# Isomorpfishm/SINGA

Measured on AMD Instinct MI355X. Metric: protein-ligand graphs/sec GAN step (G+D fwd+bwd); scatter-TP kernel HBM GB/s, higher is better.
Workload: dtype f32

## Files before the change

### __graft_entry__.py

```python
import os
import subprocess
import sys

ROOT = os.path.dirname(os.path.abspath(__file__))
if ROOT not in sys.path:
    sys.path.insert(0, ROOT)

SRC = os.path.join(ROOT, "singa_amd", "csrc", "singa_hip.hip")
LIB = os.path.join(ROOT, "singa_amd", "lib", "libsinga_hip.so")


def build() -> None:
    os.makedirs(os.path.dirname(LIB), exist_ok=True)
    deps = [SRC, os.path.join(ROOT, "singa_amd", "csrc", "so3_index.h"), os.path.join(ROOT, "include", "singa_hip.h"),
            os.path.join(ROOT, "include", "singa_hip_lab.h"), os.path.join(ROOT, "include", "singa_hip_gen.h"),
            os.path.join(ROOT, "include", "singa_hip_force.h"), os.path.join(ROOT, "include", "singa_hip_swor.h"),
            os.path.join(ROOT, "include", "singa_hip_stream.h"), os.path.join(ROOT, "include", "singa_hip_valence.h"),
            os.path.join(ROOT, "include", "singa_hip_beam.h")]
    if not os.path.exists(LIB) or any(os.path.getmtime(d) > os.path.getmtime(LIB) for d in deps):
        hipcc = os.environ.get("HIPCC", "/opt/rocm/bin/hipcc")
        cmd = [hipcc, "--offload-arch=gfx950", "-O3", "-std=c++17", "-shared", "-fPIC", "-o", LIB, SRC]
        subprocess.check_call(cmd)
    import torch
    import singa_amd
    from singa_amd import _capi
    _capi.bind(LIB)


def smoke() -> None:
    import numpy as np
    import torch

    build()
    from oracle import singa_oracle as O
    from singa_amd import graph as G
    from singa_amd.config import load_config
    from singa_amd.model.GAN import SINGA
    from tests.helpers import golden, state_from_spec

    assert torch.cuda.is_available(), "smoke() needs a GPU"
    L = 2
    dev = "cuda:0"
    sd = state_from_spec(f"singa_L{L}")
    z = golden(f"singa_L{L}_B3.npz")
    names = ["3wi2_4tpp", "4agq_5a7b", "5cp5_4nue"]
    batch = G.collate([G.load_npz(os.path.join(ROOT, "tests", "golden", f"graph_{n}.npz"), with_lap=False) for n in names])
    batch.nodes[G.PA]["lap_pe"], batch.nodes[G.LA]["lap_pe"] = torch.tensor(z["lap_p"]), torch.tensor(z["lap_l"])
    batch.extras["edge_rot_mat"] = {k: torch.tensor(z[f"rot_{k}"]) for k in ("pp", "ll", "lp")}
    batch.extras["knn"] = {G.PA: torch.tensor(z["knn_p"]), G.LA: torch.tensor(z["knn_l"])}
    batch = batch.to(dev)
    model = SINGA(load_config(lmax=L), device=dev)
    model.load_state_dict(sd, strict=False)
    model.eval()
    logits = model(batch)
    loss = torch.nn.functional.cross_entropy(logits, batch["ligand_data"]["smiIndices_tgt"].reshape(-1))
    loss.backward()
    torch.cuda.synchronize()
    og = O.collate([O.load_graph_npz(os.path.join(ROOT, "tests", "golden", f"graph_{n}.npz")) for n in names])
    rots = {k: torch.as_tensor(z[f"rot_{k}"]) for k in ("pp", "ll", "lp")}
    with torch.no_grad():
        ref = O.singa_forward(sd, og, rots, L, torch.as_tensor(z["knn_p"]), torch.as_tensor(z["knn_l"]),
                              torch.as_tensor(z["lap_p"]), torch.as_tensor(z["lap_l"]))
    err = float((logits.detach().cpu().double() - ref.double()).norm() / ref.double().norm())
    gn = float(torch.sqrt(sum((p.grad.double() ** 2).sum() for p in model.parameters() if p.grad is not None)))
    print(f"smoke: loss {float(loss):.6f} (reference {float(z['loss']):.6f}), logits rel err vs oracle {err:.2e}, "
          f"grad norm {gn:.4f} (reference {float(z['grad_total']):.4f})")
    assert err < 1e-4, err
    assert abs(gn - float(z["grad_total"])) < 1e-4 * float(z["grad_total"])


if __name__ == "__main__":
# ... 4 lines not shown
```

### singa_amd/_capi.py

```python
import ctypes as C

P = C.c_void_p
I32 = C.c_int
I64 = C.c_int64
F32 = C.c_float


class Seg(C.Structure):
    _fields_ = [("ptr", P), ("ld", I64), ("rows", C.c_int32)]


SegArr = Seg * 3


class Gemm(C.Structure):
    _fields_ = [("a", P), ("b", P), ("c", P), ("bias", P), ("lda", I64), ("ldb", I64), ("ldc", I64), ("I", C.c_int32),
                ("J", C.c_int32), ("R", C.c_int32), ("a_group", C.c_int32), ("b_group", C.c_int32), ("c_group", C.c_int32),
                ("a_group_ld", I64), ("b_group_ld", I64), ("c_group_ld", I64), ("c_split_stride", I64), ("mask", P),
                ("addend", P), ("relu", C.c_int32), ("asum", P), ("asum_stride", I64)]


class CGemm(C.Structure):
    _fields_ = [("a", P), ("b", P), ("c", P), ("lda", I64), ("ldb", I64), ("ldc", I64), ("a_im", I64), ("b_im", I64),
                ("c_im", I64), ("c_split_stride", I64), ("I", C.c_int32), ("J", C.c_int32), ("R", C.c_int32),
# ... 94 lines not shown

EXPORTS = tuple(_SIGS)

_LAB_SIGS = {
    "singa_so3_skinny_variant": ([I32], I32),
    "singa_gemm_occupancy": ([I32, I32, I32], I32),
    "singa_gemm_force_cfg": ([I32], I32),
    "singa_lap_pe_fsi_min": ([I32], I32),
}
LAB_EXPORTS = tuple(_LAB_SIGS)

_GEN_SIGS = {
    "singa_sample_token_grammar": ([P, P, P, P, P, I32, I32, I32, I32, F32, I32, F32, I32, I32] + [P] * 10, I32),
    "singa_smiles_rule_host": ([P, P, P, I32, P, P], I32),
}
GEN_EXPORTS = tuple(_GEN_SIGS)

_FORCE_SIGS = {
    "singa_sample_token_forced": ([P, P, P, P, P, I32, I32, I32, I32, F32, I32, F32, I32, I32] + [P] * 12, I32),
}
FORCE_EXPORTS = tuple(_FORCE_SIGS)

U64 = C.c_uint64
_SWOR_SIGS = {
    "singa_swor_noise_host": ([U64, P, P, P, I32, P, P, P], I32),
    "singa_swor_work": ([I32, I32], C.c_longlong),
    "singa_swor_expand": ([P, P, P, P, I32, I32, I32, I32, I32, F32, U64, P, I32] + [P] * 8 + [P], I32),
    "singa_swor_select": ([P, P, P, P, P, I32, I32, I32, I32, I32, I32, I32] + [P] * 13 + [P], I32),
    "singa_swor_follow": ([P] * 8 + [I32] * 6 + [I64] * 4 + [P], I32),
}
SWOR_EXPORTS = tuple(_SWOR_SIGS)

_STREAM_SIGS = {
    "singa_dec_self_attn_rows": ([P] * 10 + [I32, I32, P, F32, P], I32),
    "singa_sample_token_stream": ([P] * 6 + [I32, I32, I32, I32, I32, F32, I32, F32, I32, I32] + [P] * 7 + [P], I32),
    "singa_stream_refill": ([I32] * 8 + [P] * 8 + [P], I32),
    "singa_stream_refill_host": ([I32] * 8 + [P] * 8, I32),
}
STREAM_EXPORTS = tuple(_STREAM_SIGS)

_VALENCE_SIGS = {
    "singa_sample_token_valence": ([P] * 7 + [I32, I32, I32, I32, I32, F32, I32, F32, I32, I32] + [P] * 12 + [P], I32),
    "singa_valence_rule_host": ([P] * 5 + [I32] + [P] * 3, I32),
}
VALENCE_EXPORTS = tuple(_VALENCE_SIGS)

_BEAM_SIGS = {
    "singa_beam_work": ([I32, I32], C.c_longlong),
    "singa_beam_expand": ([P] * 5 + [I32] * 5 + [P] * 5 + [P], I32),
    "singa_beam_select": ([P] * 4 + [I32] * 7 + [P] * 18 + [P], I32),
}
BEAM_EXPORTS = tuple(_BEAM_SIGS)


def bind(path):
    import torch
    lib = C.CDLL(path)
    for name, (args, res) in list(_SIGS.items()) + list(_LAB_SIGS.items()) + list(_GEN_SIGS.items()) + \
            list(_FORCE_SIGS.items()) + list(_SWOR_SIGS.items()) + list(_STREAM_SIGS.items()) + list(_VALENCE_SIGS.items()) + \
            list(_BEAM_SIGS.items()):
        fn = getattr(lib, name)
        fn.argtypes = args
        fn.restype = res
    return lib


def segs(items):
    arr = SegArr()
    for i, (p, ld, rows) in enumerate(items):
        arr[i].ptr, arr[i].ld, arr[i].rows = p, ld, rows
    return arr, len(items)


def check(lib, code, what):
    if code != 0:
        raise RuntimeError(f"{what} failed ({code}): {lib.singa_last_error_string().decode()}")
```

### singa_amd/csrc/singa_hip.hip

```cpp
#include <hip/hip_runtime.h>
#include <hip/hip_ext.h>

#include <math.h>
#include <stdint.h>
#include <stdio.h>
#include <string.h>
#include <type_traits>

#include "../../include/singa_hip.h"
#include "../../include/singa_hip_lab.h"
#include "../../include/singa_hip_gen.h"
#include "../../include/singa_hip_force.h"
#include "../../include/singa_hip_swor.h"
#include "../../include/singa_hip_stream.h"
#include "../../include/singa_hip_valence.h"
#include "../../include/singa_hip_beam.h"
#include "so3_index.h"

namespace {

thread_local char g_err[256] = "ok";

int fail(int code, const char* msg) {
    snprintf(g_err, sizeof(g_err), "%s", msg);
    return code;
}

int check_launch(const char* what) {
    hipError_t e = hipGetLastError();
    if (e != hipSuccess) {
        snprintf(g_err, sizeof(g_err), "%s: %s", what, hipGetErrorString(e));
        return (int)e;
    }
    return SINGA_OK;
}

struct ProfRec {
    hipEvent_t a, b;
    int E, N, tag;
};
constexpr int PROF_CAP = 8192;
ProfRec g_prof[PROF_CAP];
int g_prof_n = 0;
bool g_prof_on = false;
unsigned long long* g_stamp_buf = nullptr;
int g_stamp_cap = 0;
__global__ void stamp_kernel(unsigned long long* dst) { *dst = (unsigned long long)wall_clock64(); }
int g_prof_edges_hint = 0;

#ifndef SINGA_KEEP_VGPR
#define SINGA_KEEP_VGPR(x) __asm__ volatile("" : "+v"(x))
#endif

#define SINGA_LAUNCH(tag_, E_, N_, kern, grid, block, st, ...)                                                   \
    do {                                                                                                          \
        if (g_prof_on && g_prof_n < PROF_CAP) {                                                                   \
            ProfRec& r_ = g_prof[g_prof_n++];                                                                     \
            (void)hipEventCreate(&r_.a);                                                                          \
            (void)hipEventCreate(&r_.b);                                                                          \
            r_.E = (E_);                                                                                          \
            r_.N = (N_);                                                                                          \
            r_.tag = (tag_);                                                                                      \
            hipExtLaunchKernelGGL(kern, grid, block, 0, (st), r_.a, r_.b, 0, __VA_ARGS__);                        \
        } else if (g_stamp_buf && 2 * (g_prof_n + 2) <= g_stamp_cap && g_prof_n + 1 < PROF_CAP) {                 \
            if (g_prof_n == 0) {                                                                                  \
                g_prof[0].a = g_prof[0].b = nullptr;                                                              \
                g_prof[0].E = g_prof[0].N = g_prof[0].tag = 0;                                                    \
                hipLaunchKernelGGL(stamp_kernel, dim3(1), dim3(1), 0, (st), g_stamp_buf);                         \
                hipLaunchKernelGGL(stamp_kernel, dim3(1), dim3(1), 0, (st), g_stamp_buf + 1);                     \
// ... 5712 lines not shown
    return SINGA_OK;
}

template <int MAXC>
__global__ __launch_bounds__(256) void knn_graph_kernel(const float* __restrict__ pos, const int* __restrict__ batch,
                                                        const long long* __restrict__ ptr, int B, int N, int k,
                                                        long long* __restrict__ row, long long* __restrict__ col) {
    const int lane = threadIdx.x & 63;
    const int i = blockIdx.x * (blockDim.x >> 6) + (threadIdx.x >> 6);
    if (i >= N) return;
    const int g = batch[i];
    long long* ro = row + (long long)i * k;
    long long* co = col + (long long)i * k;
    if (g < 0 || g >= B) {
        for (int r = lane; r < k; r += 64) ro[r] = co[r] = -1;
        return;
    }
    const int lo = (int)ptr[g], hi = (int)ptr[g + 1];
    const float px = pos[3 * i], py = pos[3 * i + 1], pz = pos[3 * i + 2];
    const unsigned long long NONE = ~0ull;
    unsigned long long key[MAXC];
#pragma unroll
    for (int t = 0; t < MAXC; ++t) {
        const int c = lo + lane + 64 * t;
        key[t] = NONE;
        if (c < hi && c != i) {
            const float dx = __fsub_rn(px, pos[3 * c]), dy = __fsub_rn(py, pos[3 * c + 1]), dz = __fsub_rn(pz, pos[3 * c + 2]);
            const float d2 = __fadd_rn(__fadd_rn(__fmul_rn(dx, dx), __fmul_rn(dy, dy)), __fmul_rn(dz, dz));
            key[t] = ((unsigned long long)__float_as_uint(d2) << 32) | (unsigned)c;
        }
    }
    for (int r = 0; r < k; ++r) {
        unsigned long long best = key[0];
#pragma unroll
        for (int t = 1; t < MAXC; ++t) best = key[t] < best ? key[t] : best;
#pragma unroll
        for (int o = 32; o > 0; o >>= 1) {
            const unsigned blo = (unsigned)__shfl_xor((int)(unsigned)best, o, 64);
            const unsigned bhi = (unsigned)__shfl_xor((int)(unsigned)(best >> 32), o, 64);
            const unsigned long long other = ((unsigned long long)bhi << 32) | blo;
            best = other < best ? other : best;
        }
#pragma unroll
        for (int t = 0; t < MAXC; ++t)
            if (key[t] == best) key[t] = NONE;
        if (lane == 0) {
            const bool have = best != NONE;
            ro[r] = have ? (long long)i : -1;
            co[r] = have ? (long long)(unsigned)best : -1;
        }
    }
}

__global__ void calib_copy_kernel(const float* __restrict__ src, float* __restrict__ dst, long long n) {
    long long i = (long long)blockIdx.x * blockDim.x + threadIdx.x;
    long long stride = (long long)gridDim.x * blockDim.x;
    for (; i < n; i += stride) dst[i] = src[i];
}

template <int UNROLL>
__global__ void __launch_bounds__(256) calib_copy16_kernel(const float4* __restrict__ src, float4* __restrict__ dst, long long n4) {
    const long long chunk = 256LL * UNROLL;
    for (long long base = (long long)blockIdx.x * chunk; base < n4; base += (long long)gridDim.x * chunk) {
        float4 v[UNROLL];
#pragma unroll
        for (int u = 0; u < UNROLL; ++u) {
            const long long i = base + threadIdx.x + 256LL * u;
            if (i < n4) v[u] = src[i];
        }
#pragma unroll
        for (int u = 0; u < UNROLL; ++u) {
            const long long i = base + threadIdx.x + 256LL * u;
            if (i < n4) dst[i] = v[u];
        }
    }
}

}

extern "C" {

int singa_prof_enable(int on) {
    g_prof_on = on != 0;
    return SINGA_OK;
}

int singa_prof_stamps(unsigned long long* buf, int cap) {
    g_stamp_buf = buf;
    g_stamp_cap = buf ? cap : 0;
    if (buf) {
        g_prof_on = false;
        g_prof_n = 0;
    }
    return SINGA_OK;
}

int singa_prof_read_stamps(const unsigned long long* host_stamps, float* ms, int* tags, int* edges, int* nodes, int cap) {
    if (!host_stamps) return 0;
    int n = 0;
    double calib = (double)(host_stamps[1] - host_stamps[0]);
    for (int i = 1; i < g_prof_n && n < cap; ++i) {
        double ticks = (double)(host_stamps[2 * i + 1] - host_stamps[2 * i]) - calib;
        ms[n] = (float)(ticks * 1e-5);
        tags[n] = g_prof[i].tag;
        edges[n] = g_prof[i].E;
        nodes[n] = g_prof[i].N;
// ... 26 lines not shown
        (void)hipEventDestroy(g_prof[i].a);
        (void)hipEventDestroy(g_prof[i].b);
    }
    g_prof_n = 0;
    return n;
}

int singa_prof_collect_tagged(float* ms, int* tags, int* edges, int* nodes, int cap) {
    int n = 0;
    for (int i = 0; i < g_prof_n; ++i) {
        float t = 0.f;
        hipError_t e = hipEventElapsedTime(&t, g_prof[i].a, g_prof[i].b);
        if (e == hipSuccess && n < cap) {
            ms[n] = t;
            tags[n] = g_prof[i].tag;
            edges[n] = g_prof[i].E;
            nodes[n] = g_prof[i].N;
            ++n;
        }
        (void)hipEventDestroy(g_prof[i].a);
        (void)hipEventDestroy(g_prof[i].b);
    }
    g_prof_n = 0;
    return n;
}

int singa_calib_copy(const float* src, float* dst, long long n, void* stream) {
    if (!src || !dst) return fail(SINGA_E_NULL, "calib_copy: null pointer");
    hipLaunchKernelGGL(calib_copy_kernel, dim3(256 * 8), dim3(256), 0, (hipStream_t)stream, src, dst, n);
    return check_launch("calib_copy");
}

int singa_knn_graph(const float* pos, const int32_t* batch, const long long* ptr, int B, int N, int k, int max_nodes, long long* row,
                    long long* col, void* stream) {
    if (!pos || !batch || !ptr || !row || !col) return fail(SINGA_E_NULL, "knn_graph: null pointer");
    if (B < 0 || N < 0 || k <= 0 || max_nodes < 0 || max_nodes > 2048) return fail(SINGA_E_SHAPE, "knn_graph: k > 0 and at most 2048 atoms per molecule");
    if (N == 0) return SINGA_OK;
    const dim3 grid((unsigned)((N + 3) / 4)), block(256);
    hipStream_t st = (hipStream_t)stream;
    if (max_nodes <= 512) hipLaunchKernelGGL(knn_graph_kernel<8>, grid, block, 0, st, pos, batch, ptr, B, N, k, row, col);
    else if (max_nodes <= 1024) hipLaunchKernelGGL(knn_graph_kernel<16>, grid, block, 0, st, pos, batch, ptr, B, N, k, row, col);
    else hipLaunchKernelGGL(knn_graph_kernel<32>, grid, block, 0, st, pos, batch, ptr, B, N, k, row, col);
    return check_launch("knn_graph");
}

int singa_knn_edge_attr(const float* len, const int32_t* ptr, long long n_real, const float* offset, float coeff, float* out, int N,
                        int G, void* stream) {
    if (!ptr || !offset || !out || (!len && n_real > 0)) return fail(SINGA_E_NULL, "knn_edge_attr: null pointer");
    if (G != 64) return fail(SINGA_E_SHAPE, "knn_edge_attr: 64 Gaussians (the shipped edge_channels)");
    if (N < 0 || n_real < 0) return fail(SINGA_E_SHAPE, "knn_edge_attr: negative size");
    if (N == 0) return SINGA_OK;
    hipLaunchKernelGGL(knn_edge_attr_kernel, dim3(kn_grid(N)), dim3(64), 0, (hipStream_t)stream, len, ptr, n_real, offset, coeff, out, N);
    return check_launch("knn_edge_attr");
}

int singa_calib_copy16(const float* src, float* dst, long long n, int blocks, int unroll, void* stream) {
    if (!src || !dst) return fail(SINGA_E_NULL, "calib_copy16: null pointer");
    if (n % 4 || ((uintptr_t)src | (uintptr_t)dst) % 16) return fail(SINGA_E_SHAPE, "calib_copy16: n % 4 == 0 and 16-byte aligned pointers");
    if (blocks < 1 || blocks > (1 << 20) || (unroll != 1 && unroll != 2 && unroll != 4 && unroll != 8))
        return fail(SINGA_E_SHAPE, "calib_copy16: blocks >= 1, unroll in {1, 2, 4, 8}");
    const float4* s4 = (const float4*)src;
    float4* d4 = (float4*)dst;
    hipStream_t st = (hipStream_t)stream;
    if (unroll == 1) hipLaunchKernelGGL(calib_copy16_kernel<1>, dim3(blocks), dim3(256), 0, st, s4, d4, n / 4);
    else if (unroll == 2) hipLaunchKernelGGL(calib_copy16_kernel<2>, dim3(blocks), dim3(256), 0, st, s4, d4, n / 4);
    else if (unroll == 4) hipLaunchKernelGGL(calib_copy16_kernel<4>, dim3(blocks), dim3(256), 0, st, s4, d4, n / 4);
    else hipLaunchKernelGGL(calib_copy16_kernel<8>, dim3(blocks), dim3(256), 0, st, s4, d4, n / 4);
    return check_launch("calib_copy16");
}

int singa_version(void) { return 100; }

const char* singa_last_error_string(void) { return g_err; }

int singa_init(const double* jd_flat, int lmax_max) {
    if (!jd_flat) return fail(SINGA_E_NULL, "singa_init: jd_flat is null");
    if (lmax_max < 0 || lmax_max > 11) return fail(SINGA_E_LMAX, "singa_init: lmax_max must be in [0, 11]");
    static float host[MAX_J];
    int n = j_off(lmax_max + 1);
    for (int i = 0; i < n; ++i) host[i] = (float)jd_flat[i];
    hipError_t e = hipMemcpyToSymbol(HIP_SYMBOL(g_J), host, n * sizeof(float), 0, hipMemcpyHostToDevice);
    if (e != hipSuccess) {
        snprintf(g_err, sizeof(g_err), "singa_init: %s", hipGetErrorString(e));
        return (int)e;
    }
    g_lmax_init = lmax_max;
    return SINGA_OK;
}

int singa_dims(int lmax, int mmax, int* kr, int* wsz, int* rad_rows) {
    SINGA_DISPATCH_L(lmax, mmax, {
        using I = SO3Idx<L_, 2>;
        if (kr) *kr = I::KR;
        if (wsz) *wsz = I::WSZ;
        if (rad_rows) *rad_rows = I::RAD_ROWS;
    });
    return SINGA_OK;
}

int singa_edge_frames(const float* vec, const float* rnd, float* rot, float* stats, int E, void* stream) {
    if (!vec || !rnd || !rot || !stats) return fail(SINGA_E_NULL, "edge_frames: null pointer");
    if (E <= 0) return SINGA_OK;
    hipLaunchKernelGGL(edge_frames_kernel, dim3((E + 255) / 256), dim3(256), 0, (hipStream_t)stream, vec, rnd, rot,
                       (int*)stats, E);
    return check_launch("edge_frames");
}
// ... 1463 lines not shown
```

### singa_amd/model/CProMG.py

```python
import math
import os

import numpy as np
import torch
import torch.nn as nn
import torch.nn.functional as F
from torch.nn import BatchNorm1d, Conv1d, Dropout, Embedding, LayerNorm, Sequential

from .. import ops
from ..nn import Linear


class ShiftedSoftplus(nn.Module):
    def __init__(self, device="cuda"):
        super().__init__()
        self.shift = math.log(2.0)

    def forward(self, x):
        return F.softplus(x) - self.shift


class GaussianSmearing(nn.Module):
    def __init__(self, start=0.0, stop=10.0, num_gaussians=50, device="cuda"):
        super().__init__()
# ... 1 lines not shown
        self.coeff = -0.5 / (offset[1] - offset[0]).item() ** 2
        self.register_buffer("offset", offset)

    def forward(self, dist):
        dist = dist.view(-1, 1) - self.offset.view(1, -1)
        return torch.exp(self.coeff * torch.pow(dist, 2))


class DenseMap:

    def __init__(self, batch, batch_size, mx=None):
        inside = batch < batch_size
        bc = batch.clamp(max=batch_size)
        num = torch.zeros(batch_size + 1, dtype=torch.int64, device=batch.device).index_add_(0, bc, torch.ones_like(batch))
        num = num[:batch_size]
        self.B = batch_size
        self.mx = int(num.max()) if mx is None else int(mx)
        start = num.cumsum(0) - num
        self.ptr = torch.cat([start, start[-1:] + num[-1:]])
        trash = batch_size * self.mx
        bi = batch.clamp(max=batch_size - 1)
        self.idx = torch.where(inside, torch.arange(batch.numel(), device=batch.device) - start[bi] + bi * self.mx,
                               torch.full_like(batch, trash))
        self.gidx = torch.where(inside, self.idx, torch.zeros_like(self.idx))
        mask = torch.zeros(trash + 1, dtype=torch.bool, device=batch.device)
        mask[self.idx] = True
        self.mask = mask[:trash].view(batch_size, self.mx)
        self.pad_mask = ~self.mask.unsqueeze(1)

    def tensors(self):
        return [self.idx, self.gidx, self.mask, self.pad_mask]

    def dense(self, x):
        out = x.new_zeros((self.B * self.mx + 1,) + tuple(x.shape[1:]))
        out = out.index_copy(0, self.idx, x)
        return out[:self.B * self.mx].view(self.B, self.mx, *x.shape[1:])

    def gather(self, dense_flat):
        return dense_flat.index_select(0, self.gidx)


def to_dense_batch(x, batch, batch_size):
    dm = DenseMap(batch, batch_size)
    return dm.dense(x), dm.mask, dm.idx


def knn_graph(pos, k, batch, batch_size, dm=None):
    dm = dm or DenseMap(batch, batch_size)
    return ops.knn_graph(pos, k, batch, dm.ptr, dm.mx)


class KnnEdges:

    def __init__(self, pos, knn_ei, smear, cap=None, n_real=None):
        N = pos.shape[0]
        dev = pos.device
        valid = (knn_ei[0] >= 0) & (knn_ei[1] >= 0)
        a, b = knn_ei[0].clamp(min=0), knn_ei[1].clamp(min=0)
        ln = (pos[a] - pos[b]).norm(dim=1)
        sentinel = N * N
        fwd = torch.where(valid, a * N + b, torch.full_like(a, sentinel))
        bwd = torch.where(valid, b * N + a, torch.full_like(a, sentinel))
        skey, perm = torch.sort(torch.cat([fwd, bwd]))
        new = torch.ones_like(skey, dtype=torch.bool)
        new[1:] = skey[1:] != skey[:-1]
        gid = torch.cumsum(new, 0) - 1
        triple = ((~new[2:] & ~new[1:-1] & (skey[2:] != sentinel)).any() if skey.numel() > 2
                  else torch.zeros((), dtype=torch.bool, device=dev))
        n_groups, last, triple = torch.stack([gid[-1] + 1, skey[-1], triple.to(gid.dtype)]).tolist()
        n_edges = n_groups - (1 if last == sentinel else 0)
        ukey = torch.zeros(n_groups, dtype=torch.int64, device=dev).scatter_(0, gid, skey)[:n_edges]
        ln2 = torch.cat([ln, ln])[perm]
        if not triple:
            nxt = torch.cat([ln2[1:], ln2[-1:]])
            prv = torch.cat([ln2[:1], ln2[:-1]])
            has_next = torch.cat([~new[1:], new.new_zeros(1)])
            mean = torch.where(new, torch.where(has_next, 0.5 * (ln2 + nxt), ln2), 0.5 * (prv + ln2))
            ln = torch.zeros(n_groups, device=dev).scatter_(0, gid, mean)[:n_edges]
        else:
            cnt = torch.zeros(n_groups, device=dev).index_add_(0, gid, torch.ones_like(ln2))[:n_edges]
            ln = torch.zeros(n_groups, device=dev).index_add_(0, gid, ln2)[:n_edges] / cnt
        row, col = ukey // N, ukey % N
        fused = ln.is_cuda and smear.offset.numel() == 64
        ea = None if fused else smear(ln)
        self.n_edges = n_edges + N
        if cap is not None:
            extra = cap - self.n_edges
            nd = N - n_real
            if extra < 0 or nd < 2:
                raise OverflowError(f"KnnEdges: {self.n_edges} edges do not fit the capacity {cap}")
            i = torch.arange(extra, device=dev)
            ps = (i * nd) // max(extra, 1)
            row = torch.cat([row, n_real + ps])
            col = torch.cat([col, n_real + (ps + 1 + i % (nd - 1)) % nd])
            if not fused:
                ea = torch.cat([ea, ea.new_zeros(extra, ea.shape[1])])
        loop = torch.arange(N, device=dev)
        bounds = torch.arange(N + 1, device=dev)
        if ln.is_cuda:
            E0 = row.shape[0]
            seg_ptr = torch.searchsorted(row, bounds)
            order = torch.empty(E0 + N, dtype=torch.int64, device=dev)
            order[torch.arange(E0, device=dev) + row] = torch.arange(E0, device=dev)
            order[seg_ptr[1:] + loop] = E0 + loop
            row, col = torch.cat([row, loop]), torch.cat([col, loop])
            self.row, self.col = row[order], col[order]
            seg32 = seg_ptr.to(torch.int32)
# ... 158 lines not shown

    def forward(self, x):
        return self.dropout(x + self.pe[: x.size(0), :])


class EncoderLayer(nn.Module):
    def __init__(self, config, device="cuda"):
        super().__init__()
        self.enc_self_attn = MultiHeadAttention(config.hidden_channels, config.edge_channels, config.key_channels,
                                                config.num_heads, device=device)
        self.pos_ffn = PoswiseFeedForwardNet(config.hidden_channels, device=device)

    def forward(self, node_attr, edges):
        msa_outputs = self.enc_self_attn(node_attr, edges)
        return msa_outputs, self.pos_ffn(msa_outputs)


class EncoderLayer2(nn.Module):
    def __init__(self, config, device="cuda"):
        super().__init__()
        self.enc_self_attn = MultiHeadAttention(config.hidden_channels, config.edge_channels, config.key_channels,
                                                config.num_heads, device=device)
        self.proj = Linear(config.hidden_channels, config.hidden_channels, device=device)
        self.cross_attn = MultiHeadAttention2(config.hidden_channels, config.key_channels, config.num_heads, device=device)
        self.layer_norm = LayerNorm(config.hidden_channels, device=device)
        self.pos_ffn = PoswiseFeedForwardNet(config.hidden_channels, device=device)

    def forward(self, node_attr, edges, idx, atom_msa_outputs, atom_mask, dm, before_cross=None):
        msa_outputs = self.enc_self_attn(node_attr, edges)
        if idx == 2 or idx == 5:
            if before_cross is not None:
                before_cross(idx)
            kv = self.proj(atom_msa_outputs[idx])
            cross = self.cross_attn(dm.dense(msa_outputs), kv, kv, atom_mask)
            msa_outputs = ops.layer_norm_residual(msa_outputs, dm.gather(cross.reshape(-1, cross.size(-1))), self.layer_norm)
        return self.pos_ffn(msa_outputs)


class Encoder(nn.Module):
    def __init__(self, config, protein_atom_feature_dim, device="cuda"):
        super().__init__()
        self.config = config
        self.protein_atom_emb = Linear(protein_atom_feature_dim, config.hidden_channels, device=device)
        self.laplacian_emb = Linear(config.lap_dim, config.hidden_channels, device=device)
        self.layers = nn.ModuleList([EncoderLayer(config, device=device) for _ in range(config.num_interactions)])
        self.distance_expansion = GaussianSmearing(stop=15, num_gaussians=config.edge_channels, device=device)
        self.out = Linear(config.hidden_channels, config.hidden_channels, device=device)
        self.layer_norm = LayerNorm(config.hidden_channels, device=device)

    def prepare(self, pos, batch, batch_size, knn=None, mx=None, cap=None, n_real=None):
        dm = DenseMap(batch, batch_size, mx)
        if knn is None:
            knn = knn_graph(pos, self.config.knn, batch, batch_size, dm)
        return {"dense": dm, "edges": KnnEdges(pos, knn, self.distance_expansion, cap, n_real)}

    def forward(self, protein_atom_feature, pos, batch, atom_laplacian, batch_size=None, knn=None, prep=None,
                layer_done=None):
        if prep is None:
            prep = self.prepare(pos, batch, int(batch.max()) + 1 if batch_size is None else batch_size, knn)
        dm, edges = prep["dense"], prep["edges"]
        node_attr = ops.linear_add(protein_atom_feature, self.protein_atom_emb.weight, self.protein_atom_emb.bias,
                                   self.laplacian_emb(atom_laplacian))
        msa_outputs1 = []
        for idx, layer in enumerate(self.layers):
            msa_outputs, node_attr = layer(node_attr, edges)
            msa_outputs1.append(dm.dense(msa_outputs) if idx in (2, 5) else None)
            if layer_done is not None and msa_outputs1[-1] is not None:
                layer_done(idx, msa_outputs1[-1])
        return dm.dense(node_attr), dm.pad_mask, msa_outputs1


class Encoder2(nn.Module):
    def __init__(self, config, aa_feature_dim, device="cuda"):
        super().__init__()
        self.config = config
        self.aa_emb = Linear(aa_feature_dim, config.hidden_channels, device=device)
        self.laplacian_emb = Linear(config.lap_dim, config.hidden_channels, device=device)
        self.layers = nn.ModuleList([EncoderLayer2(config, device=device) for _ in range(config.num_interactions)])
        self.distance_expansion = GaussianSmearing(stop=25, num_gaussians=config.edge_channels, device=device)
        self.out = Linear(config.hidden_channels, config.hidden_channels, device=device)
        self.layer_norm = LayerNorm(config.hidden_channels, device=device)

    def prepare(self, aa_pos, aa_batch, batch_size, knn=None, mx=None, cap=None, n_real=None):
        dm = DenseMap(aa_batch, batch_size, mx)
        if knn is None:
            knn = knn_graph(aa_pos, 30, aa_batch, batch_size, dm)
        return {"dense": dm, "edges": KnnEdges(aa_pos, knn, self.distance_expansion, cap, n_real)}

    def forward(self, aa_feature, aa_pos, aa_batch, aa_laplacian, atom_mask, atom_msa_outputs, batch_size=None, knn=None,
                prep=None, before_cross=None):
        if prep is None:
            prep = self.prepare(aa_pos, aa_batch, int(aa_batch.max()) + 1 if batch_size is None else batch_size, knn)
        dm, edges = prep["dense"], prep["edges"]
        node_attr = ops.linear_add(aa_feature, self.aa_emb.weight, self.aa_emb.bias, self.laplacian_emb(aa_laplacian))
        for idx, layer in enumerate(self.layers):
            node_attr = layer(node_attr, edges, idx, atom_msa_outputs, atom_mask, dm, before_cross)
        return dm.dense(node_attr), dm.pad_mask


class DecoderLayer(nn.Module):
    def __init__(self, config, device="cuda"):
        super().__init__()
        self.dec_self_attn = MultiHeadDeAttention(config.hidden_channels, config.key_channels, config.num_heads, device=device)
        self.dec_enc_attn = MultiHeadDeAttention(config.hidden_channels, config.key_channels, config.num_heads, device=device)
        self.pos_ffn = PoswiseFeedForwardDeNet(config.hidden_channels, device=device)

    def forward(self, dec_inputs, enc_outputs, dec_self_attn_mask, dec_enc_attn_mask):
        dec_outputs = self.dec_self_attn(dec_inputs, dec_inputs, dec_inputs, dec_self_attn_mask)
        dec_outputs = self.dec_enc_attn(dec_outputs, enc_outputs, enc_outputs, dec_enc_attn_mask)
        return self.pos_ffn(dec_outputs)


class Decoder(nn.Module):
    def __init__(self, config, num_props=None, device="cuda"):
        super().__init__()
        self.config, self.device, self.num_props = config, device, num_props
        self.mol_emb = Embedding(len(config.smiVoc), config.hidden_channels, 0, device=device)
        self.pos_emb = PositionalEncoding(config.hidden_channels, device=device)
        self.type_emb = Embedding(2, config.hidden_channels, device=device)
        if self.num_props:
            self.prop_nn = Linear(self.num_props, config.hidden_channels, device=device)
        self.layers = nn.ModuleList([DecoderLayer(config, device=device) for _ in range(config.num_interactions)])
        self.pad_id = list(config.smiVoc).index("^")

    def forward(self, smiles_index, enc_outputs, enc_pad_mask, tgt_len, prop=None):
        b, t = smiles_index.size()
        dev = smiles_index.device
        dec_inputs = ops.embedding(self.mol_emb.weight, smiles_index, self.mol_emb.padding_idx)
        dec_inputs = self.pos_emb(dec_inputs.transpose(0, 1)).transpose(0, 1)
        ids = smiles_index
        num = 0
        if self.num_props:
            assert prop.shape[-1] == self.num_props
            dec_inputs = ops.bias_add(dec_inputs, self.type_emb.weight[1])
            p = ops.bias_add(self.prop_nn(prop.unsqueeze(1)), self.type_emb.weight[0])
            dec_inputs = torch.cat([p, dec_inputs], 1)
            ids = torch.cat([torch.ones(b, 1, dtype=ids.dtype, device=dev), ids], 1)
            num = 1
        n = t + num
        pad = ids.eq(self.pad_id).unsqueeze(1).expand(b, n, n)
# ... 70 lines not shown
```

### singa_amd/ops.py

```python
import ctypes
import math
import warnings

import torch

warnings.filterwarnings("ignore", message=".*preferred_blas_library is an experimental feature.*")

from . import _capi, _lib, so3


PROFILE_ON = False


def profile_start(in_graph=False):
    global PROFILE_ON, _STAMPS
    PROFILE_ON = True
    if in_graph:
        _STAMPS = torch.zeros(2 * 8192 + 2, dtype=torch.int64, device="cuda")
        _chk(_lib.lib().singa_prof_stamps(_p(_STAMPS), _STAMPS.numel()), "singa_prof_stamps")
    else:
        _chk(_lib.lib().singa_prof_enable(1), "singa_prof_enable")


_STAMPS = None
# ... 291 lines not shown
        ctx.save_for_backward(w, v, row_ptr)
        if E == 0:
            return torch.zeros(N, H, F, device=v.device, dtype=torch.float32)
        out = torch.empty(N, H, F, device=v.device, dtype=torch.float32)
        _chk(_lib.lib().singa_segment_wsum_fwd(_p(w), _p(v), _p(row_ptr), _p(out), N, H, F, _stream()),
             "singa_segment_wsum_fwd")
        return out

    @staticmethod
    def backward(ctx, g):
        w, v, row_ptr = ctx.saved_tensors
        g = g.contiguous()
        E, H, F = v.shape
        N = row_ptr.numel() - 1
        gw, gv = torch.empty_like(w), torch.empty_like(v)
        if E == 0:
            return gw, gv, None
        _chk(_lib.lib().singa_segment_wsum_bwd(_p(g), _p(w), _p(v), _p(row_ptr), _p(gw), _p(gv), N, H, F, _stream()),
             "singa_segment_wsum_bwd")
        return gw, gv, None


def segment_sum_rows(v, row_ptr):
    v = v.detach()
    _dev(v, row_ptr)
    E, F = v.shape
    N = row_ptr.numel() - 1
    out = torch.empty(N, 1, F, device=v.device, dtype=torch.float32)
    w = torch.ones(max(E, 1), 1, device=v.device, dtype=torch.float32)
    _chk(_lib.lib().singa_segment_wsum_fwd(_p(w), _p(v), _p(row_ptr), _p(out), N, 1, F, _stream()), "singa_segment_wsum_fwd")
    return out.view(N, F)


def knn_edge_attr(ln, seg_ptr, E0, n_real, offset, coeff):
    ln, offset = ln.detach().contiguous(), offset.detach().contiguous()
    _dev(ln, seg_ptr, offset)
    N = seg_ptr.numel() - 1
    out = torch.empty(E0 + N, offset.numel(), device=ln.device, dtype=torch.float32)
    _chk(_lib.lib().singa_knn_edge_attr(_p(ln), _p(seg_ptr), int(n_real), _p(offset), float(coeff), _p(out), N, offset.numel(),
                                        _stream()), "singa_knn_edge_attr")
    return out


def knn_graph(pos, k, batch, ptr, max_nodes):
    pos = pos.detach().to(torch.float32).contiguous()
    b32 = batch.to(torch.int32).contiguous()
    _dev(pos, b32)
    p64 = ptr.to(device=pos.device, dtype=torch.int64).contiguous()
    N = pos.shape[0]
    out = torch.empty(2, N * k, dtype=torch.int64, device=pos.device)
    _chk(_lib.lib().singa_knn_graph(_p(pos), _p(b32), _p(p64), p64.numel() - 1, N, int(k), int(max_nodes), _p(out[0]), _p(out[1]),
                                    _stream()), "singa_knn_graph")
    return out


def segment_wsum(w, v, row_ptr):
    return _SegmentWSum.apply(w, v, row_ptr)


_grid_cache = {}


def _grid_factors(L, M, m_primary, device):
    key = (L, M, m_primary, str(device))
    if key not in _grid_cache:
        _grid_cache[key] = tuple(torch.tensor(t, dtype=torch.float32, device=device).contiguous()
                                 for t in so3.s2_grid_factors(L, M, m_primary))
    return _grid_cache[key]


class _S2ActEdge(torch.autograd.Function):

    @staticmethod
    def forward(ctx, h0, h1, h2, gate_off, x_off, C, L, M):
        h0, h1, h2 = _rows(h0), _rows(h1), _rows(h2)
        _dev(h0, h1, h2)
        lay = so3.layout(L, M)
        P, Q, A = _grid_factors(L, M, True, h0.device)
        E = h0.shape[0]
        out = torch.empty(E, lay.KR * C, device=h0.device, dtype=torch.float32)
        seg, n = _segs3((h0[:, x_off:], h1, h2), lay.seg_rows, C)
        _chk(_lib.lib().singa_s2act_sep_fwd(seg, n, _p(h0[:, gate_off:]), h0.stride(0), _p(P),
                                            _p(Q), _p(A), _p(out), E, C, L, _stream()), "singa_s2act_sep_fwd")
        ctx.save_for_backward(h0, h1, h2)
        ctx.cfg = (gate_off, x_off, C, L, M)
        return out

    @staticmethod
    def backward(ctx, g):
        h0, h1, h2 = ctx.saved_tensors
        gate_off, x_off, C, L, M = ctx.cfg
        lay = so3.layout(L, M)
        P, Q, A = _grid_factors(L, M, True, h0.device)
        g = g.contiguous()
        E = h0.shape[0]
        gx = torch.empty(E, lay.KR * C, device=g.device, dtype=torch.float32)
        gg = torch.empty(E, C, device=g.device, dtype=torch.float32)
        seg, n = _segs3((h0[:, x_off:], h1, h2), lay.seg_rows, C)
        _chk(_lib.lib().singa_s2act_sep_bwd(seg, n, _p(h0[:, gate_off:]), h0.stride(0), _p(P),
                                            _p(Q), _p(A), _p(g), _p(gx), _p(gg), E, C, L, _stream()),
             "singa_s2act_sep_bwd")
        n0, n1 = lay.seg_rows[0] * C, lay.seg_rows[1] * C
        g0 = torch.zeros_like(h0)
        g0[:, gate_off:gate_off + C] = gg
        g0[:, x_off:] = gx[:, :n0]
        return g0, gx[:, n0:n0 + n1], gx[:, n0 + n1:], None, None, None, None, None
# ... 1685 lines not shown
```

Before: 862.0.

## Build symmetrized kNN edge CSR on GPU with per-molecule bitset kernels

Adds HIP kernels that build the symmetrized, deduplicated kNN edge graph per molecule. Each molecule gets an LDS adjacency bitset, and the kernels count degrees, scan row pointers and fill row/col, int32 copies, the transpose permutation and the edge endpoints directly. This replaces the torch-op construction in KnnEdges (masking, sorting, unique) when inputs qualify, falling back otherwise. It adds a host sync to read the edge total and flags, and needs up to 128KB of LDS for 1024-atom molecules.

```diff
diff --git a/__graft_entry__.py b/__graft_entry__.py
--- a/__graft_entry__.py
+++ b/__graft_entry__.py
@@ -16,7 +16,7 @@
             os.path.join(ROOT, "include", "singa_hip_lab.h"), os.path.join(ROOT, "include", "singa_hip_gen.h"),
             os.path.join(ROOT, "include", "singa_hip_force.h"), os.path.join(ROOT, "include", "singa_hip_swor.h"),
             os.path.join(ROOT, "include", "singa_hip_stream.h"), os.path.join(ROOT, "include", "singa_hip_valence.h"),
-            os.path.join(ROOT, "include", "singa_hip_beam.h")]
+            os.path.join(ROOT, "include", "singa_hip_beam.h"), os.path.join(ROOT, "include", "singa_hip_knn.h")]
     if not os.path.exists(LIB) or any(os.path.getmtime(d) > os.path.getmtime(LIB) for d in deps):
         hipcc = os.environ.get("HIPCC", "/opt/rocm/bin/hipcc")
         cmd = [hipcc, "--offload-arch=gfx950", "-O3", "-std=c++17", "-shared", "-fPIC", "-o", LIB, SRC]
diff --git a/include/singa_hip_knn.h b/include/singa_hip_knn.h
--- /dev/null
+++ b/include/singa_hip_knn.h
@@ -0,0 +1,18 @@
+#ifndef SINGA_HIP_KNN_H
+#define SINGA_HIP_KNN_H
+#include <stdint.h>
+#ifdef __cplusplus
+extern "C" {
+#endif
+
+int singa_knn_csr_max_nodes(void);
+int singa_knn_csr_count(const long long* row, const long long* col, const long long* ptr, int B, int N, int k, int max_nodes, int n_real,
+                        int32_t* cnt, int32_t* flags, int32_t* row_ptr, int32_t* meta, void* stream);
+int singa_knn_csr_fill(const long long* row, const long long* col, const long long* ptr, int B, int N, int k, int max_nodes, int n_real,
+                       const int32_t* row_ptr, long long* out_row, long long* out_col, int32_t* out_row32, int32_t* out_col32,
+                       int32_t* eperm, long long* a0, long long* b0, void* stream);
+
+#ifdef __cplusplus
+}
+#endif
+#endif
diff --git a/singa_amd/_capi.py b/singa_amd/_capi.py
--- a/singa_amd/_capi.py
+++ b/singa_amd/_capi.py
@@ -170,13 +170,20 @@
 }
 BEAM_EXPORTS = tuple(_BEAM_SIGS)
 
+_KNN_SIGS = {
+    "singa_knn_csr_max_nodes": ([], I32),
+    "singa_knn_csr_count": ([P, P, P, I32, I32, I32, I32, I32, P, P, P, P, P], I32),
+    "singa_knn_csr_fill": ([P, P, P, I32, I32, I32, I32, I32] + [P] * 8 + [P], I32),
+}
+KNN_EXPORTS = tuple(_KNN_SIGS)
+
 
 def bind(path):
     import torch
     lib = C.CDLL(path)
     for name, (args, res) in list(_SIGS.items()) + list(_LAB_SIGS.items()) + list(_GEN_SIGS.items()) + \
             list(_FORCE_SIGS.items()) + list(_SWOR_SIGS.items()) + list(_STREAM_SIGS.items()) + list(_VALENCE_SIGS.items()) + \
-            list(_BEAM_SIGS.items()):
+            list(_BEAM_SIGS.items()) + list(_KNN_SIGS.items()):
         fn = getattr(lib, name)
         fn.argtypes = args
         fn.restype = res
diff --git a/singa_amd/csrc/singa_hip.hip b/singa_amd/csrc/singa_hip.hip
--- a/singa_amd/csrc/singa_hip.hip
+++ b/singa_amd/csrc/singa_hip.hip
@@ -15,6 +15,7 @@
 #include "../../include/singa_hip_stream.h"
 #include "../../include/singa_hip_valence.h"
 #include "../../include/singa_hip_beam.h"
+#include "../../include/singa_hip_knn.h"
 #include "so3_index.h"
 
 namespace {
@@ -5833,6 +5834,164 @@
     }
 }
 
+constexpr int KNN_CSR_MAX_NODES = 1024;
+#ifndef SINGA_EMUL
+enum { KCSR_BAD_CENTRE = 1, KCSR_BAD_NEIGHBOUR = 2, KCSR_REPEAT = 4, KCSR_TOO_BIG = 8, KCSR_PADDING = 16 };
+
+__device__ __forceinline__ int knn_csr_bits(unsigned* bits, const long long* __restrict__ row, const long long* __restrict__ col,
+                                            int lo, int n, int W, int k, int n_real) {
+    for (int x = threadIdx.x; x < n * W; x += blockDim.x) bits[x] = 0u;
+    __syncthreads();
+    int bad = 0;
+    for (int s = threadIdx.x; s < n * k; s += blockDim.x) {
+        const int t = s / k, q = s - t * k;
+        const long long base = (long long)(lo + t) * k;
+        const long long a = row[base + q], b = col[base + q];
+        if (a < 0 || b < 0) continue;
+        if (a != lo + t) { bad |= KCSR_BAD_CENTRE; continue; }
+        if (b < lo || b >= lo + n || b == a) { bad |= KCSR_BAD_NEIGHBOUR; continue; }
+        if (a >= n_real || b >= n_real) { bad |= KCSR_PADDING; continue; }
+        bool rep = false;
+        for (int p = 0; p < q; ++p) rep |= col[base + p] == b && row[base + p] >= 0;
+        if (rep) { bad |= KCSR_REPEAT; continue; }
+        const int u = (int)b - lo;
+        atomicOr(&bits[t * W + (u >> 5)], 1u << (u & 31));
+        atomicOr(&bits[u * W + (t >> 5)], 1u << (t & 31));
+    }
+    __syncthreads();
+    return bad;
+}
+
+__global__ void __launch_bounds__(1024) knn_csr_count_kernel(const long long* __restrict__ row, const long long* __restrict__ col,
+                                                             const long long* __restrict__ ptr, int B, int N, int k, int max_nodes,
+                                                             int n_real, int* __restrict__ cnt, int* __restrict__ flags) {
+    extern __shared__ __attribute__((aligned(16))) unsigned kcsr_bits[];
+    __shared__ int bad_all;
+    const int g = blockIdx.x, tid = threadIdx.x;
+    if (tid == 0) bad_all = 0;
+    __syncthreads();
+    int bad = 0;
+    if (g == B) {
+        for (int i = (int)ptr[B] + tid; i < N; i += blockDim.x) {
+            cnt[i] = 1;
+            for (int q = 0; q < k; ++q) bad |= (row[(long long)i * k + q] >= 0 && col[(long long)i * k + q] >= 0) ? KCSR_BAD_CENTRE : 0;
+        }
+    } else {
+        const int lo = (int)ptr[g], n = (int)ptr[g + 1] - lo;
+        if (n > max_nodes) {
+            bad = KCSR_TOO_BIG;
+            for (int t = tid; t < n; t += blockDim.x) cnt[lo + t] = 1;
+        } else if (n > 0) {
+            const int W = (n + 31) >> 5;
+            bad = knn_csr_bits(kcsr_bits, row, col, lo, n, W, k, n_real);
+            for (int t = tid; t < n; t += blockDim.x) {
+                int c = 1;
+                for (int w = 0; w < W; ++w) c += __popc(kcsr_bits[t * W + w]);
+                cnt[lo + t] = c;
+            }
+        }
+    }
+    if (bad) atomicOr(&bad_all, bad);
+    __syncthreads();
+    if (tid == 0) flags[g] = bad_all;
+}
+
+__global__ void __launch_bounds__(1024) knn_csr_scan_kernel(const int* __restrict__ cnt, const int* __restrict__ flags, int nflags, int N,
+                                                            int* __restrict__ row_ptr, int* __restrict__ meta) {
+    __shared__ int part[1024];
+    __shared__ int bad_all;
+    const int tid = threadIdx.x;
+    if (tid == 0) bad_all = 0;
+    const int chunk = (N + 1023) / 1024;
+    const int beg = min(tid * chunk, N), end = min(beg + chunk, N);
+    int s = 0;
+    for (int i = beg; i < end; ++i) s += cnt[i];
+    part[tid] = s;
+    __syncthreads();
+    for (int o = 1; o < 1024; o <<= 1) {
+        const int v = tid >= o ? part[tid - o] : 0;
+        __syncthreads();
+        part[tid] += v;
+        __syncthreads();
+    }
+    int run = part[tid] - s;
+    for (int i = beg; i < end; ++i) {
+        row_ptr[i] = run;
+        run += cnt[i];
+    }
+    int bad = 0;
+    for (int i = tid; i < nflags; i += 1024) bad |= flags[i];
+    if (bad) atomicOr(&bad_all, bad);
+    __syncthreads();
+    if (tid == 1023) {
+        row_ptr[N] = part[1023];
+        meta[0] = part[1023];
+        meta[1] = bad_all;
+    }
+}
+
+__global__ void __launch_bounds__(1024) knn_csr_fill_kernel(const long long* __restrict__ row, const long long* __restrict__ col,
+                                                            const long long* __restrict__ ptr, int B, int N, int k, int max_nodes,
+                                                            int n_real, const int* __restrict__ row_ptr, long long* __restrict__ orow,
+                                                            long long* __restrict__ ocol, int* __restrict__ orow32,
+                                                            int* __restrict__ ocol32, int* __restrict__ eperm, long long* __restrict__ a0,
+                                                            long long* __restrict__ b0) {
+    extern __shared__ __attribute__((aligned(16))) unsigned kcsr_bits[];
+    const int g = blockIdx.x, tid = threadIdx.x, lane = tid & 63, wave = tid >> 6, nwave = blockDim.x >> 6;
+    if (g == B) {
+        for (int i = (int)ptr[B] + tid; i < N; i += blockDim.x) {
+            const int p = row_ptr[i];
+            orow[p] = ocol[p] = i;
+            orow32[p] = ocol32[p] = i;
+            eperm[p] = p;
+        }
+        return;
+    }
+    const int lo = (int)ptr[g], n = (int)ptr[g + 1] - lo;
+    if (n <= 0 || n > max_nodes) return;
+    const int W = (n + 31) >> 5;
+    if (knn_csr_bits(kcsr_bits, row, col, lo, n, W, k, n_real)) return;
+    for (int t = wave; t < n; t += nwave) {
+        const int j = lo + t, base = row_ptr[j];
+        unsigned word = lane < W ? kcsr_bits[t * W + lane] : 0u;
+        const int pc = __popc(word);
+        int incl = pc;
+#pragma unroll
+        for (int o = 1; o < 64; o <<= 1) {
+            const int v = __shfl_up(incl, o, 64);
+            if (lane >= o) incl += v;
+        }
+        const int deg = __shfl(incl, 63, 64);
+        const int tw = t >> 5;
+        const unsigned lowmask = (1u << (t & 31)) - 1u;
+        const int below = __shfl(incl - pc + __popc(word & lowmask), tw, 64);
+        int q = incl - pc;
+        while (word) {
+            const int bit = __ffs((int)word) - 1;
+            word &= word - 1u;
+            const int u = lane * 32 + bit, i = lo + u, p = base + q;
+            orow[p] = j;
+            ocol[p] = i;
+            orow32[p] = j;
+            ocol32[p] = i;
+            a0[p - j] = j;
+            b0[p - j] = i;
+            const unsigned* mu = kcsr_bits + u * W;
+            int rk = __popc(mu[tw] & lowmask);
+            for (int w = 0; w < tw; ++w) rk += __popc(mu[w]);
+            eperm[base + q + (u > t ? 1 : 0)] = row_ptr[i] + rk;
+            ++q;
+        }
+        if (lane == 0) {
+            const int p = base + deg;
+            orow[p] = ocol[p] = j;
+            orow32[p] = ocol32[p] = j;
+            eperm[base + below] = p;
+        }
+    }
+}
+#endif
+
 __global__ void calib_copy_kernel(const float* __restrict__ src, float* __restrict__ dst, long long n) {
     long long i = (long long)blockIdx.x * blockDim.x + threadIdx.x;
     long long stride = (long long)gridDim.x * blockDim.x;
@@ -5965,6 +6124,63 @@
     if (N == 0) return SINGA_OK;
     hipLaunchKernelGGL(knn_edge_attr_kernel, dim3(kn_grid(N)), dim3(64), 0, (hipStream_t)stream, len, ptr, n_real, offset, coeff, out, N);
     return check_launch("knn_edge_attr");
+}
+
+int singa_knn_csr_max_nodes(void) { return KNN_CSR_MAX_NODES; }
+
+#ifndef SINGA_EMUL
+static int knn_csr_lds(const void* fn, int max_nodes, size_t* lds) {
+    *lds = (size_t)max_nodes * (size_t)((max_nodes + 31) / 32) * sizeof(unsigned);
+    if (*lds <= 64 * 1024) return SINGA_OK;
+    hipError_t e = hipFuncSetAttribute(fn, hipFuncAttributeMaxDynamicSharedMemorySize, (int)*lds);
+    return e == hipSuccess ? SINGA_OK : fail((int)e, "knn_csr: LDS size refused");
+}
+
+#endif
+
+static int knn_csr_args(const long long* row, const long long* col, const long long* ptr, int B, int N, int k, int max_nodes, int n_real) {
+    if (!row || !col || !ptr) return fail(SINGA_E_NULL, "knn_csr: null pointer");
+    if (B < 0 || N < 0 || k <= 0 || n_real < 0 || n_real > N) return fail(SINGA_E_SHAPE, "knn_csr: B, N >= 0, k > 0, 0 <= n_real <= N");
+    if (max_nodes < 1 || max_nodes > KNN_CSR_MAX_NODES) return fail(SINGA_E_SHAPE, "knn_csr: molecules of 1 .. 1024 atoms");
+    if ((long long)N * (2LL * k + 1) > 0x7fffffffLL) return fail(SINGA_E_SHAPE, "knn_csr: more than 2^31 - 1 edges");
+    return SINGA_OK;
+}
+
+int singa_knn_csr_count(const long long* row, const long long* col, const long long* ptr, int B, int N, int k, int max_nodes, int n_real,
+                        int32_t* cnt, int32_t* flags, int32_t* row_ptr, int32_t* meta, void* stream) {
+    int rc = knn_csr_args(row, col, ptr, B, N, k, max_nodes, n_real);
+    if (rc != SINGA_OK) return rc;
+    if (!cnt || !flags || !row_ptr || !meta) return fail(SINGA_E_NULL, "knn_csr_count: null pointer");
+#ifdef SINGA_EMUL
+    return fail(SINGA_E_SHAPE, "knn_csr_count: not part of the emulation build");
+#else
+    size_t lds;
+    rc = knn_csr_lds(reinterpret_cast<const void*>(knn_csr_count_kernel), max_nodes, &lds);
+    if (rc != SINGA_OK) return rc;
+    hipStream_t st = (hipStream_t)stream;
+    hipLaunchKernelGGL(knn_csr_count_kernel, dim3(B + 1), dim3(1024), lds, st, row, col, ptr, B, N, k, max_nodes, n_real, cnt, flags);
+    hipLaunchKernelGGL(knn_csr_scan_kernel, dim3(1), dim3(1024), 0, st, cnt, flags, B + 1, N, row_ptr, meta);
+    return check_launch("knn_csr_count");
+#endif
+}
+
+int singa_knn_csr_fill(const long long* row, const long long* col, const long long* ptr, int B, int N, int k, int max_nodes, int n_real,
+                       const int32_t* row_ptr, long long* out_row, long long* out_col, int32_t* out_row32, int32_t* out_col32,
+                       int32_t* eperm, long long* a0, long long* b0, void* stream) {
+    int rc = knn_csr_args(row, col, ptr, B, N, k, max_nodes, n_real);
+    if (rc != SINGA_OK) return rc;
+    if (!row_ptr || !out_row || !out_col || !out_row32 || !out_col32 || !eperm || !a0 || !b0)
+        return fail(SINGA_E_NULL, "knn_csr_fill: null pointer");
+#ifdef SINGA_EMUL
+    return fail(SINGA_E_SHAPE, "knn_csr_fill: not part of the emulation build");
+#else
+    size_t lds;
+    rc = knn_csr_lds(reinterpret_cast<const void*>(knn_csr_fill_kernel), max_nodes, &lds);
+    if (rc != SINGA_OK) return rc;
+    hipLaunchKernelGGL(knn_csr_fill_kernel, dim3(B + 1), dim3(1024), lds, (hipStream_t)stream, row, col, ptr, B, N, k, max_nodes, n_real,
+                       row_ptr, out_row, out_col, out_row32, out_col32, eperm, a0, b0);
+    return check_launch("knn_csr_fill");
+#endif
 }
 
 int singa_calib_copy16(const float* src, float* dst, long long n, int blocks, int unroll, void* stream) {
diff --git a/singa_amd/model/CProMG.py b/singa_amd/model/CProMG.py
--- a/singa_amd/model/CProMG.py
+++ b/singa_amd/model/CProMG.py
@@ -77,7 +77,56 @@
 
 class KnnEdges:
 
-    def __init__(self, pos, knn_ei, smear, cap=None, n_real=None):
+    use_csr = True
+
+    def _from_csr(self, pos, knn_ei, smear, cap, n_real, ptr, mx):
+        N = pos.shape[0]
+        dev = pos.device
+        if not (pos.is_cuda and knn_ei.is_cuda and smear.offset.numel() == 64 and N > 0):
+            return False
+        lim = N if n_real is None else int(n_real)
+        if not 0 <= lim <= N:
+            return False
+        counted = ops.knn_csr_count(knn_ei, ptr, N, int(mx), lim)
+        if counted is None or counted[2]:
+            return False
+        row_ptr, total, _ = counted
+        n_edges = total - N
+        E, extra = total, 0
+        if cap is not None:
+            extra, nd = cap - total, N - lim
+            if extra < 0 or nd < 2:
+                raise OverflowError(f"KnnEdges: {total} edges do not fit the capacity {cap}")
+            E = cap
+        row, col, row32, col32, eperm, a0, b0 = ops.knn_csr_fill(knn_ei, ptr, N, int(mx), lim, row_ptr, total, E)
+        col_ptr = row_ptr.clone()
+        if extra > 0:
+            i = torch.arange(extra, device=dev)
+            ps = (i * nd) // extra
+            p = torch.arange(nd, device=dev)
+            upto = torch.searchsorted(ps, p, right=True)
+            first = total - nd
+            epos, lpos = first + i + ps, first + upto + p
+            row[epos], col[epos] = lim + ps, lim + (ps + 1 + i % (nd - 1)) % nd
+            row[lpos], col[lpos] = lim + p, lim + p
+            row32[first:], col32[first:] = row[first:], col[first:]
+            row_ptr[lim + 1:] = first + upto + p + 1
+            order = torch.argsort(col32[first:], stable=True)
+            eperm[first:] = first + order
+            col_ptr[lim + 1:] = first + torch.searchsorted(col[first:][order], torch.arange(lim + 1, N + 1, device=dev))
+        ln = (pos[a0] - pos[b0]).norm(dim=1)
+        seg32 = row_ptr - torch.arange(N + 1, dtype=torch.int32, device=dev)
+        self.attr = ops.knn_edge_attr(ln, seg32, E - N, n_edges, smear.offset, smear.coeff)
+        self.row, self.col, self.row32, self.col32 = row, col, row32, col32
+        self.row_ptr, self.eperm, self.col_ptr = row_ptr, eperm, col_ptr
+        self.n_edges, self.N = total, N
+        return True
+
+    def __init__(self, pos, knn_ei, smear, cap=None, n_real=None, ptr=None, mx=None):
+        self.route = "torch"
+        if KnnEdges.use_csr and ptr is not None and mx is not None and self._from_csr(pos, knn_ei, smear, cap, n_real, ptr, mx):
+            self.route = "csr"
+            return
         N = pos.shape[0]
         dev = pos.device
         valid = (knn_ei[0] >= 0) & (knn_ei[1] >= 0)
@@ -342,7 +391,7 @@
         dm = DenseMap(batch, batch_size, mx)
         if knn is None:
             knn = knn_graph(pos, self.config.knn, batch, batch_size, dm)
-        return {"dense": dm, "edges": KnnEdges(pos, knn, self.distance_expansion, cap, n_real)}
+        return {"dense": dm, "edges": KnnEdges(pos, knn, self.distance_expansion, cap, n_real, dm.ptr, dm.mx)}
 
     def forward(self, protein_atom_feature, pos, batch, atom_laplacian, batch_size=None, knn=None, prep=None,
                 layer_done=None):
@@ -375,7 +424,7 @@
         dm = DenseMap(aa_batch, batch_size, mx)
         if knn is None:
             knn = knn_graph(aa_pos, 30, aa_batch, batch_size, dm)
-        return {"dense": dm, "edges": KnnEdges(aa_pos, knn, self.distance_expansion, cap, n_real)}
+        return {"dense": dm, "edges": KnnEdges(aa_pos, knn, self.distance_expansion, cap, n_real, dm.ptr, dm.mx)}
 
     def forward(self, aa_feature, aa_pos, aa_batch, aa_laplacian, atom_mask, atom_msa_outputs, batch_size=None, knn=None,
                 prep=None, before_cross=None):
diff --git a/singa_amd/ops.py b/singa_amd/ops.py
--- a/singa_amd/ops.py
+++ b/singa_amd/ops.py
@@ -367,6 +367,43 @@
     _chk(_lib.lib().singa_knn_graph(_p(pos), _p(b32), _p(p64), p64.numel() - 1, N, int(k), int(max_nodes), _p(out[0]), _p(out[1]),
                                     _stream()), "singa_knn_graph")
     return out
+
+
+def _knn_csr_args(knn_ei, ptr, N, max_nodes):
+    if (not knn_ei.is_cuda or knn_ei.dtype != torch.int64 or knn_ei.dim() != 2 or knn_ei.shape[0] != 2 or N <= 0
+            or knn_ei.shape[1] == 0 or knn_ei.shape[1] % N or not 1 <= max_nodes <= _lib.lib().singa_knn_csr_max_nodes()):
+        return None
+    k = knn_ei.shape[1] // N
+    if N * (2 * k + 1) >= 2 ** 31:
+        return None
+    p64 = ptr.to(device=knn_ei.device, dtype=torch.int64).contiguous()
+    return knn_ei[0].contiguous(), knn_ei[1].contiguous(), p64, p64.numel() - 1, k
+
+
+def knn_csr_count(knn_ei, ptr, N, max_nodes, n_real):
+    a = _knn_csr_args(knn_ei, ptr, N, max_nodes)
+    if a is None:
+        return None
+    row, col, p64, B, k = a
+    dev = row.device
+    scratch = torch.empty(N + B + 1, dtype=torch.int32, device=dev)
+    row_ptr = torch.empty(N + 1, dtype=torch.int32, device=dev)
+    meta = torch.empty(2, dtype=torch.int32, device=dev)
+    _chk(_lib.lib().singa_knn_csr_count(_p(row), _p(col), _p(p64), B, N, k, int(max_nodes), int(n_real), _p(scratch), _p(scratch[N:]),
+                                        _p(row_ptr), _p(meta), _stream()), "singa_knn_csr_count")
+    total, flags = meta.tolist()
+    return row_ptr, total, flags
+
+
+def knn_csr_fill(knn_ei, ptr, N, max_nodes, n_real, row_ptr, total, E):
+    row, col, p64, B, k = _knn_csr_args(knn_ei, ptr, N, max_nodes)
+    dev = row.device
+    orow, ocol = (torch.empty(E, dtype=torch.int64, device=dev) for _ in range(2))
+    orow32, ocol32, eperm = (torch.empty(E, dtype=torch.int32, device=dev) for _ in range(3))
+    a0, b0 = (torch.empty(max(total - N, 1), dtype=torch.int64, device=dev) for _ in range(2))
+    _chk(_lib.lib().singa_knn_csr_fill(_p(row), _p(col), _p(p64), B, N, k, int(max_nodes), int(n_real), _p(row_ptr), _p(orow), _p(ocol),
+                                       _p(orow32), _p(ocol32), _p(eperm), _p(a0), _p(b0), _stream()), "singa_knn_csr_fill")
+    return orow, ocol, orow32, ocol32, eperm, a0[:total - N], b0[:total - N]
 
 
 def segment_wsum(w, v, row_ptr):
```

Result: no change. 859.8 (-0.2%).
